# zzpDapeng/Transformer-Transducer

Hardware: AMD Instinct MI355X
Metric: utterances/sec (fwd+bwd) on 80-d fbank T=500 U=50 (higher is better)
Workload: dtype bf16

## Files before the change

### transformer-transducer_amd/csrc/gemm_fast.hip

```cpp
#include "gemm_fast.h"
#include "ttmi.h"
#include <mutex>

void ttmi_probe_begin(int slot, hipStream_t st);
void ttmi_probe_end(int slot, hipStream_t st);

namespace {

typedef float f32x16 __attribute__((ext_vector_type(16)));
typedef __bf16 bf16x8 __attribute__((ext_vector_type(8)));
typedef __bf16 bf16x4 __attribute__((ext_vector_type(4)));
typedef short s16x4 __attribute__((ext_vector_type(4)));

constexpr int TM = 128, TN_ = 128, TK = 64, NTH = 256;
constexpr int TILE_B = 128 * 64 * 2;
constexpr int GROUP_M = 8;

__device__ __attribute__((aligned(16))) const uint4 g_zero16 = {0u, 0u, 0u, 0u};

struct FP {
    const bf16_t* A;
    const bf16_t* B;
    void* C;
    const float* bias;
// ... 1622 lines not shown
        if (grp == 1) V9_BAR();
        int stg = 0;
        for (int t = 0; t < cnk; ++t) {
            const unsigned base = lds0 + stg * STG9;
#pragma unroll
            for (int ks = 0; ks < 2; ++ks) {
#pragma unroll
                for (int i = 0; i < 4; ++i) {
                    const unsigned a = base + aoff[i];
                    bf16x4 lo, hi;
                    if (ks == 0) { LDS_TR(lo, a, 0); LDS_TR(hi, a, 4 * 512); }
                    else { LDS_TR(lo, a, 32 * 512); LDS_TR(hi, a, 36 * 512); }
                    af[i][ks] = __builtin_shufflevector(lo, hi, 0, 1, 2, 3, 4, 5, 6, 7);
                }
#pragma unroll
                for (int i = 0; i < 4; ++i) {
                    const unsigned bq = base + boff[i];
                    bf16x4 lo, hi;
                    if (ks == 0) { LDS_TR(lo, bq, 0); LDS_TR(hi, bq, 4 * 256); }
                    else { LDS_TR(lo, bq, 32 * 256); LDS_TR(hi, bq, 36 * 256); }
                    bfr[i][ks] = __builtin_shufflevector(lo, hi, 0, 1, 2, 3, 4, 5, 6, 7);
                }
            }
            if (t + 2 < cnk) {
                TTMI_VM_GUARD("v9");
                stage(stg == 0 ? 2 : stg - 1, t + 2);
                TTMI_VM_WAIT("v9", V9_INFLIGHT);
            } else {
                asm volatile("s_waitcnt vmcnt(0)" ::: "memory");
            }
            asm volatile("s_waitcnt lgkmcnt(0)" ::: "memory");
            V9_BAR();
            __builtin_amdgcn_s_setprio(1);
#pragma unroll
            for (int ks = 0; ks < 2; ++ks)
#pragma unroll
                for (int mt = 0; mt < 4; ++mt)
#pragma unroll
                    for (int nt = 0; nt < 4; ++nt)
                        acc[mt][nt] = __builtin_amdgcn_mfma_f32_16x16x32_bf16(bfr[nt][ks], af[mt][ks], acc[mt][nt], 0, 0, 0);
            if (CS) {
#pragma unroll
                for (int mt = 0; mt < 4; ++mt)
#pragma unroll
                    for (int ks = 0; ks < 2; ++ks)
                        if (cs_unit == mt * 2 + ks) cs = __builtin_amdgcn_mfma_f32_16x16x32_bf16(ones, af[mt][ks], cs, 0, 0, 0);
            }
            __builtin_amdgcn_s_setprio(0);
            V9_BAR();
            stg = stg == 2 ? 0 : stg + 1;
        }
        if (grp == 0) V9_BAR();

        const int cbm = bm, cbn = bn, cunit = cs_unit;
        it += ncu;
        live = it < nitems;
        if (live) { item(it, bm, bn, tn); sources(bm, bn, kbeg); stage(0, 0); if (nk > 1) { TTMI_VM_GUARD("v9"); stage(1, 1); } }

        if (cnk > 0) {
            float* C = reinterpret_cast<float*>(p.C);
            float* img = reinterpret_cast<float*>(smem + 2 * STG9 + wave * 4096);
#pragma unroll
            for (int mi = 0; mi < 4; ++mi) {
#pragma unroll
                for (int ni = 0; ni < 4; ++ni)
                    *reinterpret_cast<f32x4*>(img + (lane & 15) * 64 + ((ni * 4 + (lane >> 4)) ^ (lane & 15)) * 4) = acc[mi][ni];
                const int n = cbn + wc * 64 + lane;
#pragma unroll
                for (int r = 0; r < 16; ++r) {
                    const int m = cbm + wr * 64 + mi * 16 + r;
                    const float v = img[r * 64 + (((lane >> 2) ^ r) << 2) + (lane & 3)];
                    if (m < p.M && n < p.N) atomicAdd(C + (long)m * p.ldc + n, v);
                }
            }
            if (CS && cunit >= 0 && lane < 16) {
                const int m = cbm + wr * 64 + (cunit >> 1) * 16 + lane;
                if (m < p.M) atomicAdd(p.colsum + m, cs[0]);
            }
        }
    }
#undef V9_BAR
}

struct TnGroupProb {
    const bf16_t* A; const bf16_t* B; float* C; float* colsum;
    int M, N, K, tiles_m;
    long lda, ldb, ldc;
    int tile0;
};
struct TnGroup {
    TnGroupProb pr[16];
    int n, total;
    int pieces;
};

__global__ __launch_bounds__(NTH8, 1) void gemm_tn_bf16_group_kernel(const TnGroup g) {
    extern __shared__ __attribute__((aligned(16))) char smem[];
    const unsigned lds0 = (unsigned)(size_t)smem;
    const int tid = threadIdx.x, lane = tid & 63, wave = __builtin_amdgcn_readfirstlane(tid >> 6);
    const int wr = wave & 3, wc = wave >> 2;
    const int grp = wave >> 2;
    const int xcd = blockIdx.x & 7, cu = blockIdx.x >> 3, ncu = gridDim.x >> 3;
    const int per_x = (g.total + 7) / 8;
    const int lo_x = min(xcd * per_x, g.total), hi = min((xcd + 1) * per_x, g.total);
    const int n_x = hi - lo_x, n_rounds = n_x / ncu, n_sur = n_x - n_rounds * ncu;
    const int P = (g.pieces && n_sur > 0 && 2 * n_sur <= ncu) ? ncu / n_sur : 0;
    const int n_whole = P ? n_rounds * ncu : n_x;
    const int n_items = n_whole + (P ? n_sur * P : 0);

    unsigned oA[4], oB[2];
    const char* baseA = nullptr;
    const char* baseB = nullptr;
    long lda = 0, ldb = 0;
    int nk = 0, q = 0;
    bool piece = false;
    auto item = [&](int v, int& bm, int& bn, int& tn) {
        piece = v >= n_whole;
        const int it = lo_x + (piece ? n_whole + (v - n_whole) / P : v);
        q = 0;
        while (q + 1 < g.n && it >= g.pr[q + 1].tile0) ++q;
        const TnGroupProb& pr = g.pr[q];
        const int t = it - pr.tile0;
        bm = (t % pr.tiles_m) * T9M;
        tn = t / pr.tiles_m;
        bn = tn * T9N;
        lda = pr.lda; ldb = pr.ldb;
        nk = pr.K / TK;
        baseA = reinterpret_cast<const char*>(pr.A);
        baseB = reinterpret_cast<const char*>(pr.B);
        if (piece) {
            const int part = (v - n_whole) % P;
            const long k0 = (long)part * nk / P, k1 = (long)(part + 1) * nk / P;
            baseA += k0 * TK * lda * 2;
            baseB += k0 * TK * ldb * 2;
            nk = (int)(k1 - k0);
        }
#pragma unroll
        for (int j = 0; j < 4; ++j) {
            const int k = (wave * 4 + j) * 2 + (lane >> 5);
            const int c = (lane & 31) ^ (((k & 3) << 2) | (((k >> 3) & 1) << 1));
            oA[j] = (unsigned)((k * lda + bm + c * 8) * 2);
        }
#pragma unroll
        for (int j = 0; j < 2; ++j) {
            const int k = (wave * 2 + j) * 4 + (lane >> 4);
            const int c = (lane & 15) ^ (((k & 3) << 2) | (((k >> 3) & 1) << 1));
            oB[j] = (unsigned)((k * ldb + bn + c * 8) * 2);
        }
    };
    auto stage = [&](int stg, int kt) {
        char* dst = smem + stg * STG9;
        const char* ba = baseA + (long)kt * TK * lda * 2;
        const char* bb = baseB + (long)kt * TK * ldb * 2;
#pragma unroll
        for (int j = 0; j < 4; ++j) glds16(ba + oA[j], dst + (wave * 4 + j) * 1024);
#pragma unroll
        for (int j = 0; j < 2; ++j) glds16(bb + oB[j], dst + T9M * 128 + (wave * 2 + j) * 1024);
    };

    const int gq = lane >> 4, qq = (lane >> 2) & 3, pp = lane & 3;
    const int swz = (qq << 2) | ((gq & 1) << 1);
    int aoff[4], boff[4];
#pragma unroll
    for (int i = 0; i < 4; ++i) {
        const int ca = wr * 64 + i * 16 + 4 * pp, cb = wc * 64 + i * 16 + 4 * pp;
        aoff[i] = (gq * 8 + qq) * 512 + (((ca >> 3) ^ swz) << 4) + (ca & 7) * 2;
        boff[i] = T9M * 128 + (gq * 8 + qq) * 256 + (((cb >> 3) ^ swz) << 4) + (cb & 7) * 2;
    }
    f32x4 acc[4][4];
    f32x4 cs = {0.f, 0.f, 0.f, 0.f};
    bf16x8 af[4][2], bfr[4][2];
    bf16x8 ones;
#pragma unroll
    for (int i = 0; i < 8; ++i) ones[i] = (__bf16)1.0f;
#define V9_BAR() __builtin_amdgcn_s_barrier()

    int bm = 0, bn = 0, tn = 0;
    int it = cu;
    bool live = it < n_items;
    if (live) { item(it, bm, bn, tn); stage(0, 0); if (nk > 1) { TTMI_VM_GUARD("v9"); stage(1, 1); } }
    while (live) {
#pragma unroll
        for (int i = 0; i < 4; ++i)
#pragma unroll
            for (int j = 0; j < 4; ++j) acc[i][j] = f32x4{0.f, 0.f, 0.f, 0.f};
        cs = f32x4{0.f, 0.f, 0.f, 0.f};
        const TnGroupProb cur = g.pr[q];
        const bool cpiece = piece;
        const int cs_mt = (cur.colsum && tn < 2) ? __builtin_amdgcn_readfirstlane(tn * 2 + wc) : -1;
        const int cnk = nk;
        if (cnk > 1) TTMI_VM_WAIT("v9", V9_INFLIGHT);
        else asm volatile("s_waitcnt vmcnt(0)" ::: "memory");
        V9_BAR();
        if (grp == 1) V9_BAR();
        int stg = 0;
        for (int t = 0; t < cnk; ++t) {
            const unsigned base = lds0 + stg * STG9;
#pragma unroll
            for (int ks = 0; ks < 2; ++ks) {
#pragma unroll
                for (int i = 0; i < 4; ++i) {
                    const unsigned a = base + aoff[i];
                    bf16x4 lo, hi2;
                    if (ks == 0) { LDS_TR(lo, a, 0); LDS_TR(hi2, a, 4 * 512); }
                    else { LDS_TR(lo, a, 32 * 512); LDS_TR(hi2, a, 36 * 512); }
                    af[i][ks] = __builtin_shufflevector(lo, hi2, 0, 1, 2, 3, 4, 5, 6, 7);
                }
#pragma unroll
                for (int i = 0; i < 4; ++i) {
                    const unsigned bq = base + boff[i];
                    bf16x4 lo, hi2;
                    if (ks == 0) { LDS_TR(lo, bq, 0); LDS_TR(hi2, bq, 4 * 256); }
                    else { LDS_TR(lo, bq, 32 * 256); LDS_TR(hi2, bq, 36 * 256); }
                    bfr[i][ks] = __builtin_shufflevector(lo, hi2, 0, 1, 2, 3, 4, 5, 6, 7);
                }
            }
            if (t + 2 < cnk) {
                TTMI_VM_GUARD("v9");
                stage(stg == 0 ? 2 : stg - 1, t + 2);
                TTMI_VM_WAIT("v9", V9_INFLIGHT);
            } else {
                asm volatile("s_waitcnt vmcnt(0)" ::: "memory");
            }
            asm volatile("s_waitcnt lgkmcnt(0)" ::: "memory");
            V9_BAR();
            __builtin_amdgcn_s_setprio(1);
#pragma unroll
            for (int ks = 0; ks < 2; ++ks)
#pragma unroll
                for (int mt = 0; mt < 4; ++mt)
#pragma unroll
                    for (int nt = 0; nt < 4; ++nt)
                        acc[mt][nt] = __builtin_amdgcn_mfma_f32_16x16x32_bf16(bfr[nt][ks], af[mt][ks], acc[mt][nt], 0, 0, 0);
#pragma unroll
            for (int mt = 0; mt < 4; ++mt)
                if (cs_mt == mt) {
                    cs = __builtin_amdgcn_mfma_f32_16x16x32_bf16(ones, af[mt][0], cs, 0, 0, 0);
                    cs = __builtin_amdgcn_mfma_f32_16x16x32_bf16(ones, af[mt][1], cs, 0, 0, 0);
                }
            __builtin_amdgcn_s_setprio(0);
// ... 356 lines not shown
    }
    int S = 1;
    bool strip_in = false;
    const bool tn8 = nbatch == 1 && accumulate && tn_v8_eligible(M, N, K, colsum_a != nullptr, &S, &strip_in);
    TTMI_REQUIRE(!colsum_w || tn8, "gemm_tn_bf16: weighted column sums exist on the persistent 256x256 kernel only (M=%d N=%d K=%d)", M, N, K);
    if (tn8) {
        const int ncu_x = g_num_cus / 8;
        p.tiles_m = M / T8; p.tiles_n = N / T8;
        const int nkt = cdiv(K, TK);
        const int Mfull = strip_in ? M : M / T8 * T8;
        p.M = Mfull; p.N = N; p.K = K; p.lda = lda; p.ldb = ldb; p.ldc = ldc;
        p.splitk = S; p.ksteps = cdiv(nkt, 8 * S); p.atomic = 1; p.gm = strip_in ? ncu_x / p.tiles_n : 0;
        if (colsum_a && p.csw) {
            if (int rc = enable_lds(gemm_tn_bf16_v8_kernel<2>, LDS8T)) return rc;
            hipLaunchKernelGGL(gemm_tn_bf16_v8_kernel<2>, dim3((unsigned)g_num_cus), dim3(NTH8), LDS8T, st, p);
        } else if (colsum_a) {
            if (int rc = enable_lds(gemm_tn_bf16_v8_kernel<1>, LDS8T)) return rc;
            hipLaunchKernelGGL(gemm_tn_bf16_v8_kernel<1>, dim3((unsigned)g_num_cus), dim3(NTH8), LDS8T, st, p);
        } else {
            if (int rc = enable_lds(gemm_tn_bf16_v8_kernel<0>, LDS8T)) return rc;
            hipLaunchKernelGGL(gemm_tn_bf16_v8_kernel<0>, dim3((unsigned)g_num_cus), dim3(NTH8), LDS8T, st, p);
        }
        TTMI_LAUNCH_CHECK("gemm_tn_bf16_v8_kernel");
        if (Mfull == M) return TTMI_OK;
        A += Mfull; C += (long)Mfull * ldc; M -= Mfull;
        if (colsum_a) colsum_a += Mfull;
        p.A = A; p.C = C; p.colsum = colsum_a;
    }
    p.M = M; p.N = N; p.K = K; p.lda = lda; p.ldb = ldb; p.ldc = ldc;
    p.tiles_m = cdiv(M, TM); p.tiles_n = cdiv(N, TN_);
    const long tiles = (long)p.tiles_m * p.tiles_n;
    const int ksteps_total = cdiv(K, TK);
    int splitk = 1;
    if (tiles * nbatch < 1024) {
        const long target = tiles * nbatch <= 16 && ksteps_total < 1024 ? std::min(g_tn_target_blocks, 256) : g_tn_target_blocks;
        splitk = (int)((target + tiles * nbatch - 1) / (tiles * nbatch));
        if (ksteps_total >= 1024 && splitk < 8) splitk = 8;
        if (splitk > ksteps_total / 4) splitk = ksteps_total / 4;
        if (splitk < 1) splitk = 1;
    }
    if (splitk >= 8) splitk = splitk / 8 * 8;
    p.ksteps = cdiv(ksteps_total, splitk);
    if (splitk < 8) splitk = cdiv(ksteps_total, p.ksteps);
    p.splitk = splitk;
    p.atomic = (splitk > 1 || accumulate) ? 1 : 0;
    p.gm = GROUP_M;
#define TN_LAUNCH(NB, CSF) hipLaunchKernelGGL((gemm_tn_bf16_kernel<NB, CSF>), dim3((unsigned)(tiles * splitk), nbatch), dim3(NTH), 2 * NB * TILE_B, st, p)
        if (g_gemm_fast_version >= 4) {
            if (colsum_a) TN_LAUNCH(1, true);
            else TN_LAUNCH(1, false);
        } else {
            if (colsum_a) TN_LAUNCH(2, true);
            else TN_LAUNCH(2, false);
        }
#undef TN_LAUNCH
    TTMI_LAUNCH_CHECK("gemm_tn_bf16_kernel");
    return TTMI_OK;
}

void gemm_fast_set_version(int v) {
    if (v == 14 || v == 15) { g_nt_stores = v == 15; return; }
    if (v >= 16) { g_bf16_mid = v - 16; return; }
    g_gemm_fast_version = v;
}
void gemm_fast_set_tn_target(int n) { g_tn_target_blocks = n; }
void gemm_fast_set_f32(int on) { g_f32_fast = on; }
int gemm_fast_f32_mode() { return g_f32_fast; }
void gemm_fast_set_reserved_cus(int n) { g_reserved_cus = n < 0 ? 0 : n; }
void gemm_fast_set_tn_group_pieces(int on) { g_tn_group_pieces = on; }
void gemm_fast_stream_reserve_cus(hipStream_t st, int n) {
    int dev = 0;
    (void)hipGetDevice(&dev);
    std::lock_guard<std::mutex> lock(g_res_mu);
    if (StreamRes* e = res_entry(dev, st, true)) { e->n = n < 0 ? 0 : n; e->has_n = true; }
}
void gemm_fast_alias_stream(hipStream_t child, hipStream_t parent) {
    int dev = 0;
    (void)hipGetDevice(&dev);
    std::lock_guard<std::mutex> lock(g_res_mu);
    if (StreamRes* e = res_entry(dev, child, true)) e->parent = parent;
}

bool gemm_tn_group_fits(const TnProblem& q) {
    return q.A && q.B && q.C && q.M > 0 && q.N > 0 && q.M % T9M == 0 && q.N % T9N == 0 && q.K % TK == 0 && q.K >= 2 * TK && q.lda % 8 == 0 && q.ldb % 8 == 0 && q.lda >= q.M && q.ldb >= q.N && q.ldc >= q.N &&
           aligned16(q.A) && aligned16(q.B) && (!q.colsum || q.N / T9N >= 2) && (long)q.K * q.lda * 2 < (1L << 32) && (long)q.K * q.ldb * 2 < (1L << 32);
}
int gemm_tn_bf16_group(const TnProblem* probs, int n, hipStream_t st) {
    TTMI_REQUIRE(probs && n >= 0, "gemm_tn_bf16_group: bad arguments");
    if (g_num_cus == 0) {
        int dev = 0, cnt = 0;
        if (hipGetDevice(&dev) == hipSuccess && hipDeviceGetAttribute(&cnt, hipDeviceAttributeMultiprocessorCount, dev) == hipSuccess && cnt > 0)
            g_num_cus = cnt / 8 * 8;
        if (g_num_cus <= 0) g_num_cus = 256;
    }
    if (int rc = enable_lds(gemm_tn_bf16_group_kernel, LDS9)) return rc;
    TnGroup g;
    g.n = 0; g.total = 0; g.pieces = 0;
    int min_nkt = 1 << 30;
    const int reserved = reserved_cus(st);
    const int cus = std::max(8, (g_num_cus - reserved) / 8 * 8);
    auto flush = [&]() -> int {
        if (g.n == 0) return TTMI_OK;
        g.pieces = reserved > 0 && min_nkt >= 2 * (cus / 8) && g_tn_group_pieces;
        min_nkt = 1 << 30;
        const bool probe = g.total >= 128;
        if (probe) ttmi_probe_begin(4, st);
        hipLaunchKernelGGL(gemm_tn_bf16_group_kernel, dim3((unsigned)cus), dim3(NTH8), LDS9, st, g);
        if (probe) ttmi_probe_end(4, st);
        TTMI_LAUNCH_CHECK("gemm_tn_bf16_group_kernel");
        g.n = 0; g.total = 0;
        return TTMI_OK;
    };
    for (int i = 0; i < n; ++i) {
        const TnProblem& q = probs[i];
        if (!gemm_tn_group_fits(q)) {
            if (int rc = gemm_tn_bf16(q.A, q.B, q.C, q.M, q.N, q.K, q.lda, q.ldb, q.ldc, 1, st, q.colsum)) return rc;
            continue;
        }
        TnGroupProb& d = g.pr[g.n];
        d.A = q.A; d.B = q.B; d.C = q.C; d.colsum = q.colsum; d.M = q.M; d.N = q.N; d.K = q.K; d.tiles_m = q.M / T9M;
        d.lda = q.lda; d.ldb = q.ldb; d.ldc = q.ldc; d.tile0 = g.total;
        g.total += d.tiles_m * (q.N / T9N);
        min_nkt = std::min(min_nkt, q.K / TK);
        if (++g.n == 16) { if (int rc = flush()) return rc; }
    }
    return flush();
}

extern "C" {
int ttmi_wgrad_group(const ttmi_wgrad_desc* descs, int n, void* stream) {
    static_assert(sizeof(ttmi_wgrad_desc) == sizeof(TnProblem), "ttmi_wgrad_desc and TnProblem must share one layout");
    return gemm_tn_bf16_group(reinterpret_cast<const TnProblem*>(descs), n, static_cast<hipStream_t>(stream));
}
int ttmi_gemm_nt_bf16(const void* A, const void* B, void* C, int c_dtype, const float* bias, int M, int N, int K, long lda,
                      long ldb, long ldc, void* stream) {
    NtEpilogue e;
    e.bias = bias;
    return gemm_nt_bf16(static_cast<const bf16_t*>(A), static_cast<const bf16_t*>(B), C, c_dtype, e, M, N, K, lda, ldb, ldc,
                        static_cast<hipStream_t>(stream), FastBatch());
}
int ttmi_gemm_nt_bf16_two_term(const void* A, const void* B, const void* B_lo, void* C, int c_dtype, const float* bias, int relu, int M, int N, int K,
                               long lda, long ldb, long ldc, void* stream) {
    NtEpilogue e;
    e.bias = bias; e.relu = relu; e.B_lo = static_cast<const bf16_t*>(B_lo);
    return gemm_nt_bf16(static_cast<const bf16_t*>(A), static_cast<const bf16_t*>(B), C, c_dtype, e, M, N, K, lda, ldb, ldc,
                        static_cast<hipStream_t>(stream), FastBatch());
}
int ttmi_gemm_nt_bf16_two_term_klo(const void* A, const void* B, const void* B_lo, void* C, int c_dtype, const float* bias, int relu, int M, int N, int K,
                                   int k_lo, long lda, long ldb, long ldc, void* stream) {
    NtEpilogue e;
    e.bias = bias; e.relu = relu; e.B_lo = static_cast<const bf16_t*>(B_lo); e.K_lo = k_lo;
    return gemm_nt_bf16(static_cast<const bf16_t*>(A), static_cast<const bf16_t*>(B), C, c_dtype, e, M, N, K, lda, ldb, ldc,
                        static_cast<hipStream_t>(stream), FastBatch());
}
int ttmi_gemm_nt_bf16_exp(const void* A, const void* B, void* C, const float* bias, float* rowsum, int nparts, const float* shift, int M, int N, int K,
                          long lda, long ldb, long ldc, void* stream) {
    NtEpilogue e;
    e.bias = bias; e.rowsum = rowsum; e.nparts = nparts; e.exp_shift = shift;
    return gemm_nt_bf16(static_cast<const bf16_t*>(A), static_cast<const bf16_t*>(B), C, 1, e, M, N, K, lda, ldb, ldc,
                        static_cast<hipStream_t>(stream), FastBatch());
}
int ttmi_gemm_nt_bf16_rowscale(const void* A, const void* B, void* C, void* mask, const float* rowscale, int M, int N, int K, long lda, long ldb, long ldc,
                               void* stream) {
    NtEpilogue e;
    e.mask = static_cast<const bf16_t*>(mask); e.mask_mode = 1; e.rowscale = rowscale;
    return gemm_nt_bf16(static_cast<const bf16_t*>(A), static_cast<const bf16_t*>(B), C, 1, e, M, N, K, lda, ldb, ldc,
                        static_cast<hipStream_t>(stream), FastBatch());
}
int ttmi_gemm_tn_bf16(const void* A, const void* B, float* C, int M, int N, int K, long lda, long ldb, long ldc, int accumulate,
                      float* colsum_a, void* stream) {
    return gemm_tn_bf16(static_cast<const bf16_t*>(A), static_cast<const bf16_t*>(B), C, M, N, K, lda, ldb, ldc, accumulate,
                        static_cast<hipStream_t>(stream), colsum_a, FastBatch());
}
int ttmi_gemm_tn_bf16_wsum(const void* A, const void* B, float* C, int M, int N, int K, long lda, long ldb, long ldc, float* colsum_a,
                           const void* colsum_w, void* stream) {
    return gemm_tn_bf16(static_cast<const bf16_t*>(A), static_cast<const bf16_t*>(B), C, M, N, K, lda, ldb, ldc, 1,
                        static_cast<hipStream_t>(stream), colsum_a, FastBatch(), static_cast<const bf16_t*>(colsum_w));
}
}
```

### transformer-transducer_amd/csrc/layers.hip

```cpp
#include "gemm.h"
#include "ttmi.h"
#include "rowops.h"
#include "gemm_fast.h"
#include "attn_flash.h"
#include <mutex>
#include <unordered_map>

void ttmi_probe_begin(int slot, hipStream_t st);
void ttmi_probe_end(int slot, hipStream_t st);
void ttmi_rnnt_set_lattice_version(int v);
void ttmi_rnnt_set_align_debug(int v);

namespace {

constexpr int NT_ = GEMM_A_KMAJOR | GEMM_B_KMAJOR;
constexpr int NN_ = GEMM_A_KMAJOR;
constexpr int TN_ = 0;

inline size_t al4(size_t n) { return (n + 3) & ~size_t(3); }

GemmDesc mk(const float* A, const float* B, float* C, int M, int N, int K, long lda, long ldb, long ldc, int flags, int prec) {
    GemmDesc d;
    d.A = A; d.B = B; d.C = C; d.M = M; d.N = N; d.K = K; d.lda = lda; d.ldb = ldb; d.ldc = ldc;
    d.flags = flags | (prec == 1 ? GEMM_BF16_MFMA : (prec == 2 ? GEMM_BF16X3 : 0));
// ... 854 lines not shown
    TTMI_REQUIRE(dz && y && w1 && w2 && ln_g && ctx && ws && (dy || skip_pre_norm) && g_w1 && g_b1 && g_w2 && g_b2 && g_ln_g && g_ln_b,
                 "ffn_bwd: null pointer");
    hipStream_t st = static_cast<hipStream_t>(stream);
    const bool fast = ffn_fast(prec, d, Di);
    TTMI_REQUIRE(!out || (fast && keep && aligned16(keep)), "ffn_bwd_defer: bf16 pipeline and a 16-byte aligned keep buffer required");
    Bump bc(const_cast<float*>(ctx)), bw(ws);
    FfnCtx c(bc, rows, d, Di, fast);
    FfnWs w(bw, rows, d, Di, fast, keep);
    DropSpec d_out, d_layer;
    d_out.p = p_drop; d_out.seed = seed ^ 0xC3u; d_out.salt = g_drop_salt;
    d_layer.p = p_layer; d_layer.seed = seed ^ 0xD4u; d_layer.salt = g_drop_salt;
    const float inv_keep = 1.f / (1.f - p_drop);
    CK(ln_bwd(dz, c.s2, c.mean2, c.rstd2, ln_g, nullptr, rows, d, w.dres, g_ln_g, g_ln_b, st, d_layer, fast ? w.dres16 : nullptr, d_out,
              fast ? g_b2 : nullptr));
    const float* df = w.dres;
    if (!fast) {
        if (p_drop > 0.f) {
            CK(dropout_apply(w.dres, rows * d, d_out, w.f, nullptr, st));
            df = w.f;
        }
        CK(colsum(df, d, rows, d, 1, 1, 0, 0, 0, 0, g_b2, st));
    }
    if (fast) {
        bf16_t* a1 = static_cast<bf16_t*>(c.a1);
        bf16_t* h = static_cast<bf16_t*>(c.h);
        bf16_t* da1 = static_cast<bf16_t*>(w.da1);
        int rc = TTMI_OK;
        const bf16_t* w1T16 = ctx_weightT(ctx, 0, w1, Di, d, Di, c.w1T16, st, &rc);
        CK(rc);
        const bf16_t* w2T16 = ctx_weightT(ctx, 1, w2, d, Di, d, c.w2T16, st, &rc);
        CK(rc);
        ctx_forget(ctx);
        if (out) out[0] = ttmi_wgrad_desc{w.dres16, a1, g_w2, nullptr, d, Di, (int)rows, (long)d, (long)Di, (long)Di};
        else CK(gemm_tn_bf16(w.dres16, a1, g_w2, d, Di, (int)rows, d, Di, Di, 1, fork_stream(st)));
        NtEpilogue e;
        e.mask = a1; e.scale = inv_keep;
        CK(gemm_nt_bf16(w.dres16, w2T16, da1, 1, e, (int)rows, Di, d, d, d, Di, st));
        if (out) out[1] = ttmi_wgrad_desc{da1, h, g_w1, g_b1, Di, d, (int)rows, (long)Di, (long)d, (long)d};
        else CK(gemm_tn_bf16(da1, h, g_w1, Di, d, (int)rows, Di, d, d, 1, fork_stream(st), g_b1));
        CK(gemm_nt_bf16(da1, w1T16, w.dh, 0, nullptr, (int)rows, d, Di, Di, Di, d, st));
    } else {
        const float* a1 = static_cast<const float*>(c.a1);
        const float* h = static_cast<const float*>(c.h);
        float* da1 = static_cast<float*>(w.da1);
        bf16_t* x3 = prec == 2 ? reinterpret_cast<bf16_t*>(ws + ((bw.floats() + 63) & ~(size_t)63)) : nullptr;
        if (x3 && x3_worth(rows, Di, d)) {
            CK(x3_tn(df, a1, g_w2, d, Di, rows, d, Di, Di, x3, st));
            CK(x3_nn(df, w2, da1, (int)rows, Di, d, d, Di, Di, NtEpilogue(), x3, st, true));
            CK(relu_mask_scale(da1, a1, rows * Di, inv_keep, st));
            CK(colsum(da1, Di, rows, Di, 1, 1, 0, 0, 0, 0, g_b1, st));
            CK(x3_tn(da1, h, g_w1, Di, d, rows, Di, d, d, x3, st));
            CK(x3_nn(da1, w1, w.dh, (int)rows, d, Di, Di, d, d, NtEpilogue(), x3, st, true));
        } else {
        CK(wgrad(df, a1, g_w2, d, Di, (int)rows, d, Di, Di, prec, st));
        GemmDesc g = mk(df, w2, da1, (int)rows, Di, d, d, Di, Di, NN_ | GEMM_MASK_AUX, prec);
        g.aux = a1; g.alpha = inv_keep;
        CK(ttmi_launch_gemm(g, st));
        CK(colsum(da1, Di, rows, Di, 1, 1, 0, 0, 0, 0, g_b1, st));
        CK(wgrad(da1, h, g_w1, Di, d, (int)rows, Di, d, d, prec, st));
        CK(ttmi_launch_gemm(mk(da1, w1, w.dh, (int)rows, d, Di, Di, d, d, NN_, prec), st));
        }
    }
    if (!skip_pre_norm) CK(ln_bwd(w.dh, y, c.mean1, c.rstd1, ln_g, w.dres, rows, d, dy, g_ln_g, g_ln_b, st));
    join_stream(st);
    return TTMI_OK;
}

int ttmi_ffn_bwd(const float* dz, const float* y, const float* w1, const float* w2, const float* ln_g, long rows, int d, int Di,
                 int prec, float p_drop, float p_layer, unsigned seed, const float* ctx, float* ws, float* dy, float* g_w1,
                 float* g_b1, float* g_w2, float* g_b2, float* g_ln_g, float* g_ln_b, void* stream) {
    return ffn_bwd_impl(dz, y, w1, w2, ln_g, rows, d, Di, prec, p_drop, p_layer, seed, ctx, ws, dy, g_w1, g_b1, g_w2, g_b2, g_ln_g, g_ln_b,
                        nullptr, nullptr, stream);
}
size_t ttmi_ffn_bwd_keep_bytes(long rows, int d, int Di) { return 2 * (keep_al((size_t)rows * Di) + keep_al((size_t)rows * d)); }
int ttmi_ffn_bwd_defer(const float* dz, const float* y, const float* w1, const float* w2, const float* ln_g, long rows, int d, int Di,
                       int prec, float p_drop, float p_layer, unsigned seed, const float* ctx, float* ws, float* dy, float* g_w1,
                       float* g_b1, float* g_w2, float* g_b2, float* g_ln_g, float* g_ln_b, void* keep, ttmi_wgrad_desc* out,
                       void* stream) {
    TTMI_REQUIRE(keep && out, "ffn_bwd_defer: keep buffer and descriptor array required");
    return ffn_bwd_impl(dz, y, w1, w2, ln_g, rows, d, Di, prec, p_drop, p_layer, seed, ctx, ws, dy, g_w1, g_b1, g_w2, g_b2, g_ln_g, g_ln_b,
                        keep, out, stream);
}
int ttmi_wgrad_defer_supported(long rows, int d, int H, int Dh, int Di, int prec) {
    return rows > 0 && attn_fast(prec, d, H, Dh) && ffn_fast(prec, d, Di) ? 1 : 0;
}

static size_t ws_round(size_t floats) { return (floats + 63) & ~size_t(63); }
int ttmi_layer_fused(int d, int H, int Dh, int Di, int prec) {
    return attn_fast(prec, d, H, Dh) && ffn_fast(prec, d, Di) && ln_bwd_pair_supported(d) ? 1 : 0;
}
size_t ttmi_layer_ws_floats(int B, int L, int d, int H, int Dh, int Di, int prec) {
    return ws_round(ttmi_attn_ws_floats(B, L, d, H, Dh, prec)) + ws_round(ttmi_ffn_ws_floats((long)B * L, d, Di, prec)) + ws_round((size_t)B * L * d) + 64;
}

int ttmi_layer_fwd(const float* x, const void* x16_in, const float* qkv_w, const float* o_w, const float* ln_g, const float* ln_b, const float* r_emb,
                   const float* r_w_bias, const float* r_bias, const float* w1, const float* b1, const float* w2, const float* b2,
                   const float* ff_ln_g, const float* ff_ln_b, int B, int L, int d, int H, int Dh, int K, int Di, int mask_kind, int mask_left,
                   int mask_right, const unsigned char* mask, long mask_sb, long mask_si, int prec, float p_drop_attn, unsigned seed_attn,
                   float p_drop_ffn, float p_layer, unsigned seed_ffn, float* ctx_attn, float* ctx_ffn, float* ws, float* y, float* z,
                   void* z16_out, void* stream) {
    TTMI_REQUIRE(ctx_attn && ctx_ffn && ws && y && z && ff_ln_g && ff_ln_b, "layer_fwd: null pointer");
    TTMI_REQUIRE(B > 0 && L > 0 && d > 0 && H > 0 && Dh > 0 && Di > 0, "layer_fwd: bad dims");
    TTMI_REQUIRE((reinterpret_cast<uintptr_t>(ctx_ffn) & 255) == 0, "layer_fwd: ctx_ffn must be 256-byte aligned");
    const bool fuse = ttmi_layer_fused(d, H, Dh, Di, prec) != 0;
    TTMI_REQUIRE(fuse || (!x16_in && !z16_out), "layer_fwd: bf16 copies of the residual stream exist in the fused bf16 pipeline only (ttmi_layer_fused)");
    const long rows = (long)B * L;
    float* ws_ffn = ws + ws_round(ttmi_attn_ws_floats(B, L, d, H, Dh, prec));
    LnPreNorm pre;
    if (fuse) {
        Bump bc(ctx_ffn);
        FfnCtx fc(bc, rows, d, Di, true);
        pre.g = ff_ln_g; pre.b = ff_ln_b; pre.h16 = static_cast<bf16_t*>(fc.h); pre.mean = fc.mean1; pre.rstd = fc.rstd1;
    }
    CK(attn_fwd_impl(x, qkv_w, o_w, ln_g, ln_b, r_emb, r_w_bias, r_bias, B, L, d, H, Dh, K, mask_kind, mask_left, mask_right, mask, mask_sb, mask_si,
                     prec, p_drop_attn, seed_attn, ctx_attn, ws, y, static_cast<const bf16_t*>(x16_in), fuse ? &pre : nullptr, stream));
    return ffn_fwd_impl(y, w1, b1, w2, b2, ff_ln_g, ff_ln_b, rows, d, Di, prec, p_drop_ffn, p_layer, seed_ffn, ctx_ffn, ws_ffn, z, fuse,
                        static_cast<bf16_t*>(z16_out), stream);
}

int ttmi_layer_bwd(const float* dz, const float* x, const void* x16_in, const float* y, const float* qkv_w, const float* o_w, const float* ln_g,
                   const float* r_emb, const float* r_w_bias, const float* r_bias, const float* w1, const float* w2, const float* ff_ln_g, int B,
                   int L, int d, int H, int Dh, int K, int Di, int mask_kind, int mask_left, int mask_right, const unsigned char* mask,
                   long mask_sb, long mask_si, int prec, float p_drop_attn, unsigned seed_attn, float p_drop_ffn, float p_layer,
                   unsigned seed_ffn, const float* ctx_attn, const float* ctx_ffn, float* ws, float* dx, float* g_qkv_w, float* g_o_w,
                   float* g_ln_g, float* g_ln_b, float* g_r_emb, float* g_r_w_bias, float* g_r_bias, float* g_w1, float* g_b1, float* g_w2,
                   float* g_b2, float* g_ff_ln_g, float* g_ff_ln_b, void* keep_attn, void* keep_ffn, ttmi_wgrad_desc* out, void* stream) {
    TTMI_REQUIRE(dz && x && y && ctx_attn && ctx_ffn && ws && dx, "layer_bwd: null pointer");
    TTMI_REQUIRE(B > 0 && L > 0 && d > 0 && H > 0 && Dh > 0 && Di > 0, "layer_bwd: bad dims");
    TTMI_REQUIRE((!out && !keep_attn && !keep_ffn) || (out && keep_attn && keep_ffn), "layer_bwd: keep buffers and descriptors come together");
    const bool fuse = ttmi_layer_fused(d, H, Dh, Di, prec) != 0;
    TTMI_REQUIRE(fuse || !x16_in, "layer_bwd: a bf16 copy of x exists in the fused bf16 pipeline only");
    const long rows = (long)B * L;
    float* ws_ffn = ws + ws_round(ttmi_attn_ws_floats(B, L, d, H, Dh, prec));
    float* dy = ws_ffn + ws_round(ttmi_ffn_ws_floats(rows, d, Di, prec));
    CK(ffn_bwd_impl(dz, y, w1, w2, ff_ln_g, rows, d, Di, prec, p_drop_ffn, p_layer, seed_ffn, ctx_ffn, ws_ffn, fuse ? nullptr : dy, g_w1, g_b1, g_w2,
                    g_b2, g_ff_ln_g, g_ff_ln_b, keep_ffn, out, stream, fuse));
    LnPairIn pair;
    if (fuse) {
        Bump bc(const_cast<float*>(ctx_ffn)), bw(ws_ffn);
        FfnCtx fc(bc, rows, d, Di, true);
        FfnWs fw(bw, rows, d, Di, true, keep_ffn);
        pair = LnPairIn{fw.dh, y, fc.mean1, fc.rstd1, ff_ln_g, fw.dres, g_ff_ln_g, g_ff_ln_b};
    }
    return attn_bwd_impl(fuse ? nullptr : dy, x, qkv_w, o_w, ln_g, r_emb, r_w_bias, r_bias, B, L, d, H, Dh, K, mask_kind, mask_left, mask_right, mask,
                         mask_sb, mask_si, prec, p_drop_attn, seed_attn, ctx_attn, ws, dx, g_qkv_w, g_o_w, g_ln_g, g_ln_b, g_r_emb, g_r_w_bias,
                         g_r_bias, keep_attn, out ? out + 2 : nullptr, stream, static_cast<const bf16_t*>(x16_in), fuse ? &pair : nullptr);
}

static inline bool joint_fast(int prec, int J) { return prec == 1 && J % 8 == 0; }
static inline size_t al8(size_t n) { return (n + 7) & ~(size_t)7; }
static inline bool joint_input_fast(int prec, int B, int T, int U1, int de, int dd, int J) {
    if (!joint_fast(prec, J) || de % 8 || dd % 8 || (long)B * T < 1024) return false;
    const size_t M = (size_t)B * T * U1, din = (size_t)de + dd;
    const size_t need = al8((size_t)B * T * de) + al8((size_t)B * U1 * dd) + al8((size_t)B * T * J) + 2 * al8((size_t)B * U1 * J) + al8(din * J) + 8;
    return need <= (size_t)M * J && need + al8(din * J) + al8((size_t)B * U1 * dd) <= 2 * (size_t)M * J;
}
int ttmi_joint_logits_dtype(int prec, int J) { return joint_fast(prec, J) ? 1 : 0; }

size_t ttmi_joint_ctx_floats(int B, int T, int U1, int J) { return al4(((size_t)B * T * U1 + 63) / 64 * 64 * J); }
size_t ttmi_joint_ctx_floats_prec(int B, int T, int U1, int J, int prec) {
    const size_t f = ttmi_joint_ctx_floats(B, T, U1, J);
    if (prec != 2) return f;
    const size_t x = al4((size_t)B * T * U1 * x3_pad(J) + 64);
    return x > f ? x : f;
}
static bool joint_x3_h3(long M, int V, int J) { return x3_worth(M, V, J) && J % 4 == 0; }
size_t ttmi_joint_ws_floats(int B, int T, int U1, int J, int V) {
// ... 423 lines not shown
```

### transformer-transducer_amd/tt/transformer.py

```python
import os

import torch
import torch.nn as nn

from ttmi import ops
from ttmi.ops import MaskSpec


def default_precision():
    v = os.environ.get("TTMI_PRECISION", "fp32").lower()
    return 1 if v in ("bf16", "1") else (2 if v in ("bf16x3", "2") else 0)


def label_precision():
    if default_precision() != 1:
        return None
    v = os.environ.get("TTMI_LABEL_PRECISION", "").lower()
    return 2 if v in ("bf16x3", "2") else (0 if v in ("fp32", "0") else None)


def label_value_precision():
    if default_precision() != 1:
        return None
    v = os.environ.get("TTMI_LABEL_VALUE_PRECISION", "bf16x3").lower()
    return 2 if v in ("bf16x3", "2") else (0 if v in ("fp32",) else None)


_mask_cache = {}


def as_mask_spec(mask, B, L):
    if mask is None:
        return MaskSpec(0)
    if isinstance(mask, MaskSpec):
        return mask
    ent = _mask_cache.get(id(mask))
    if ent is not None and ent[0]() is mask and ent[1] == mask._version:
        return ent[2]
    m = mask != 0
    if m.dim() == 2:
        t = m.t().unsqueeze(1)
    elif m.dim() == 3:
        t = m.permute(2, 0, 1)
    else:
        raise ValueError("attn_mask must be 2-D (klen, bsz) or 3-D (qlen, klen, bsz)")
    spec = MaskSpec(3, tensor=t.to(torch.uint8).contiguous())
    if t.is_cuda and t.shape[1] > 1:
        keep = ~t
        n = keep.sum(-1)
        lo = keep.int().argmax(-1)
        hi = t.shape[-1] - 1 - keep.flip(-1).int().argmax(-1)
        if bool(((n > 0) & (n == hi - lo + 1)).all()):
            rows = torch.arange(t.shape[1], device=t.device)
            reach = torch.stack([(rows - lo).max(), (hi - rows).max()]).clamp_(min=0).tolist()
            spec = MaskSpec(4, left=int(reach[0]), right=int(reach[1]), tensor=torch.stack([lo, hi], -1).to(torch.int32).contiguous())
    if len(_mask_cache) > 32:
        _mask_cache.clear()
    import weakref
    _mask_cache[id(mask)] = (weakref.ref(mask), mask._version, spec)
    return spec


def grad_targets(params, names, late=()):
    bufs, rets, after, later = {}, [], [], []
    for n, prm in zip(names, params):
        if getattr(prm, "_ttmi_direct", False) and prm.grad is not None:
            bufs[n] = prm.grad
            rets.append(None)
            cb = getattr(prm, "_ttmi_on_grad", None)
            if cb is not None:
                (later if n in late else after).append(cb)
        else:
            bufs[n] = torch.zeros_like(prm)
            rets.append(bufs[n])
    return (bufs, tuple(rets), after) if not late else (bufs, tuple(rets), after, later)


def _defer_queue(params, names, late, rows, prec, first_layer=False):
    q = ops.wgrad_queue
    if q is None or rows < 4096 or prec != 1 or (first_layer and q.immediate_first_layer):
        return None
    for n, prm in zip(names, params):
        if n in late and not (getattr(prm, "_ttmi_direct", False) and prm.grad is not None):
            return None
    return q


class _AttnFn(torch.autograd.Function):
    NAMES = ("qkv_w", "o_w", "ln_g", "ln_b", "r_emb", "r_w_bias", "r_bias")

    LATE = ("qkv_w", "o_w")

    @staticmethod
    def forward(ctx, x, qkv_w, o_w, ln_g, ln_b, r_emb, r_w_bias, r_bias, mask, prec, p_drop, seed, first_layer=False):
        x = x.contiguous()
        p = dict(zip(_AttnFn.NAMES, (t.detach() for t in (qkv_w, o_w, ln_g, ln_b, r_emb, r_w_bias, r_bias))))
        y, saved = ops.attn_fwd(x, p, mask, prec, p_drop, seed)
        ctx.save_for_backward(x, saved, *p.values())
        ctx.prec, ctx.p_drop, ctx.seed, ctx.mask, ctx.first_layer = prec, p_drop, seed, mask, first_layer
        ctx.params = (qkv_w, o_w, ln_g, ln_b, r_emb, r_w_bias, r_bias)
        return y

    @staticmethod
    def backward(ctx, dy):
        x, saved, *ps = ctx.saved_tensors
        p = dict(zip(_AttnFn.NAMES, ps))
        q = _defer_queue(ctx.params, _AttnFn.NAMES, _AttnFn.LATE, x.shape[0] * x.shape[1], ctx.prec, ctx.first_layer)
        if q is not None and ops.wgrad_defer_supported(x.shape[0] * x.shape[1], x.shape[2], p["r_emb"].shape[1], p["r_emb"].shape[2],
                                                      x.shape[2], ctx.prec):
            grads, rets, after, later = grad_targets(ctx.params, _AttnFn.NAMES, _AttnFn.LATE)
            dx = ops.attn_bwd(dy.contiguous(), x, p, saved, ctx.prec, grads, ctx.p_drop, ctx.seed, ctx.mask, defer=q)
            q.add_callbacks(later)
            q.maybe_flush(force=ctx.first_layer)
        else:
            grads, rets, after = grad_targets(ctx.params, _AttnFn.NAMES)
            dx = ops.attn_bwd(dy.contiguous(), x, p, saved, ctx.prec, grads, ctx.p_drop, ctx.seed, ctx.mask)
            if ctx.first_layer:
                ops.wgrad_flush()
        for cb in after:
            cb()
        return (dx, *rets, None, None, None, None, None)


class _FFNFn(torch.autograd.Function):
    NAMES = ("ff_w1", "ff_b1", "ff_w2", "ff_b2", "ff_ln_g", "ff_ln_b")

    @staticmethod
    def forward(ctx, y, w1, b1, w2, b2, ln_g, ln_b, prec, p_drop, p_layer, seed, first_layer=False):
        y = y.contiguous()
        p = dict(zip(_FFNFn.NAMES, (t.detach() for t in (w1, b1, w2, b2, ln_g, ln_b))))
        z, saved = ops.ffn_fwd(y, p, prec, p_drop, p_layer, seed)
        ctx.save_for_backward(y, saved, *p.values())
        ctx.prec, ctx.drop, ctx.first_layer = prec, (p_drop, p_layer, seed), first_layer
        ctx.params = (w1, b1, w2, b2, ln_g, ln_b)
        return z

    LATE = ("ff_w1", "ff_b1", "ff_w2")

    @staticmethod
    def backward(ctx, dz):
        y, saved, *ps = ctx.saved_tensors
        p = dict(zip(_FFNFn.NAMES, ps))
        rows = y.numel() // y.shape[-1]
        if ctx.first_layer and ops.wgrad_queue is not None and ops.wgrad_queue.immediate_first_layer:
            ops.wgrad_flush()
        q = _defer_queue(ctx.params, _FFNFn.NAMES, _FFNFn.LATE, rows, ctx.prec, ctx.first_layer)
        if q is not None and ops.wgrad_defer_supported(rows, y.shape[-1], 1, 8, p["ff_w1"].shape[0], ctx.prec):
            grads, rets, after, later = grad_targets(ctx.params, _FFNFn.NAMES, _FFNFn.LATE)
            dy = ops.ffn_bwd(dz.contiguous(), y, p, saved, ctx.prec, grads, *ctx.drop, defer=q)
            q.add_callbacks(later)
        else:
            grads, rets, after = grad_targets(ctx.params, _FFNFn.NAMES)
            dy = ops.ffn_bwd(dz.contiguous(), y, p, saved, ctx.prec, grads, *ctx.drop)
        for cb in after:
            cb()
        return (dy, *rets, None, None, None, None, None)


_SUBLAYER_CALLS = bool(os.environ.get("TTMI_SUBLAYER_CALLS"))


class _LayerFn(torch.autograd.Function):
    NAMES = _AttnFn.NAMES + _FFNFn.NAMES
# ... 137 lines not shown
```

### transformer-transducer_amd/ttmi/ops.py

```python
import ctypes
import math
import os
import sys

import torch

from . import check, lib

c_int, c_long, c_float, c_void_p = ctypes.c_int, ctypes.c_long, ctypes.c_float, ctypes.c_void_p


_TRACE = bool(os.environ.get("TTMI_TRACE_CALLS"))


def _trace(name, *dims):
    if _TRACE:
        print("[ttmi] %s %s stream %x" % (name, dims, torch.cuda.current_stream().cuda_stream), file=sys.stderr, flush=True)


def _p(t):
    return c_void_p(t.data_ptr()) if t is not None else c_void_p(0)


def _stream():
# ... 102 lines not shown
    return ld


def ctc_loss_fwd(logits, labels, act_lens, label_lens, blank, workspace):
    _need_cuda(logits, labels, act_lens, label_lens, workspace)
    ld = _ctc_args(logits, labels)
    B, T, V = logits.shape
    costs = torch.empty(B, dtype=torch.float32, device=logits.device)
    check(lib().ttmi_ctc_loss_fwd(_p(logits), c_long(ld), _p(labels), _p(act_lens), _p(label_lens), c_int(B), c_int(T), c_int(labels.shape[1]),
                                  c_int(V), c_int(blank), _p(workspace), _p(costs), _stream()), "ttmi_ctc_loss_fwd")
    return costs


def ctc_loss_bwd(logits, labels, act_lens, label_lens, blank, workspace, grad_out, grad_out_stride, scale, inplace=False):
    _need_cuda(logits, labels, act_lens, label_lens, workspace, grad_out)
    ld = _ctc_args(logits, labels)
    B, T, V = logits.shape
    if inplace:
        grad = logits
    elif ld == V:
        grad = torch.empty_like(logits)
    else:
        grad = torch.empty(B, T, ld, dtype=logits.dtype, device=logits.device)[..., :V]
    check(lib().ttmi_ctc_loss_bwd(_p(logits), c_long(ld), _p(labels), _p(act_lens), _p(label_lens), c_int(B), c_int(T), c_int(labels.shape[1]),
                                  c_int(V), c_int(blank), _p(workspace), _p(grad_out), c_int(grad_out_stride), c_float(scale), _p(grad),
                                  c_long(ld), _stream()), "ttmi_ctc_loss_bwd")
    return grad


def ctc_greedy(logits, act_lens, blank=0):
    _need_cuda(logits, act_lens)
    if logits.dim() != 3 or logits.dtype is not torch.float32 or row_pitch(logits) is None:
        raise ValueError("ctc_greedy: logits must be f32 [B, T, V], dense or row-padded")
    B, T, V = logits.shape
    tokens = torch.empty(B, T, dtype=torch.int32, device=logits.device)
    count = torch.empty(B, dtype=torch.int32, device=logits.device)
    check(lib().ttmi_ctc_greedy(_p(logits), c_long(row_pitch(logits)), _p(act_lens), c_int(B), c_int(T), c_int(V), c_int(blank), _p(tokens),
                                _p(count), _stream()), "ttmi_ctc_greedy")
    return tokens, count


def linear_nt(x, w, out, bias=None, prec=0, accumulate=False):
    M, K = x.shape
    N = w.shape[0]
    flags = GEMM_A_KMAJOR | GEMM_B_KMAJOR | (GEMM_BIAS if bias is not None else 0) | _PREC_FLAG[prec]
    return gemm(x, w, out, M, N, K, x.stride(0), w.stride(0), out.stride(0), flags, bias=bias, beta=1.0 if accumulate else 0.0)


def linear_nn(g, w, out, prec=0):
    M, N = g.shape
    K = w.shape[1]
    return gemm(g, w, out, M, K, N, g.stride(0), w.stride(0), out.stride(0), GEMM_A_KMAJOR | _PREC_FLAG[prec])


def linear_tn(g, x, out, prec=0, accumulate=True):
    M, N = g.shape
    K = x.shape[1]
    return gemm(g, x, out, N, K, M, g.stride(0), x.stride(0), out.stride(0) if out.dim() == 2 else 1, _PREC_FLAG[prec],
                beta=1.0 if accumulate else 0.0)


GEMM_BIAS, GEMM_RELU, GEMM_ATOMIC, GEMM_MASK_AUX, GEMM_A_KMAJOR, GEMM_B_KMAJOR, GEMM_BF16_MFMA, GEMM_BF16X3 = 1, 2, 4, 8, 16, 32, 64, 128
_DT = {torch.float32: 0, torch.bfloat16: 1}
_PREC_FLAG = {0: 0, 1: GEMM_BF16_MFMA, 2: GEMM_BF16X3}


def gemm(A, B, C, M, N, K, lda, ldb, ldc, flags, bias=None, aux=None, alpha=1.0, beta=0.0, nz1=1, nz2=1,
         sA=(0, 0), sB=(0, 0), sC=(0, 0), splitk=1):
    _need_cuda(A, B, C, bias, aux)
    check(lib().ttmi_gemm(_p(A), _p(B), _p(C), _p(bias), _p(aux), c_int(_DT[A.dtype]), c_int(_DT[B.dtype]),
                          c_int(_DT[C.dtype]), c_int(M), c_int(N), c_int(K), c_long(lda), c_long(ldb), c_long(ldc),
                          c_int(nz1), c_int(nz2), c_long(sA[0]), c_long(sA[1]), c_long(sB[0]), c_long(sB[1]),
                          c_long(sC[0]), c_long(sC[1]), c_float(alpha), c_float(beta), c_int(flags), c_int(splitk),
                          _stream()), "ttmi_gemm")
    return C


class WgradDesc(ctypes.Structure):
    _fields_ = [("A", c_void_p), ("B", c_void_p), ("C", c_void_p), ("colsum", c_void_p), ("M", c_int), ("N", c_int), ("K", c_int),
                ("lda", c_long), ("ldb", c_long), ("ldc", c_long)]


class _WgradLane:
    __slots__ = ("stream", "descs", "alive", "after")

    def __init__(self, stream):
        self.stream, self.descs, self.alive, self.after = stream, [], [], []


class WgradQueue:

    def __init__(self, group=4, immediate_first_layer=False):
        self.limit = 4 * group
        self.immediate_first_layer = immediate_first_layer
        self.lanes = {}

    def _lane(self):
        st = torch.cuda.current_stream()
        key = (st.device.index, st.cuda_stream)
        lane = self.lanes.get(key)
        if lane is None:
            lane = self.lanes[key] = _WgradLane(st)
        return lane

    @property
    def descs(self):
        return self._lane().descs

    def push(self, descs, tensors):
        lane = self._lane()
        lane.descs.extend(WgradDesc.from_buffer_copy(d) for d in descs)
        lane.alive.append(tensors)

    def add_callbacks(self, cbs):
        self._lane().after.extend(cbs)

    def maybe_flush(self, force=False):
        lane = self._lane()
        if lane.descs and (force or len(lane.descs) >= self.limit):
            arr = (WgradDesc * len(lane.descs))(*lane.descs)
            check(lib().ttmi_wgrad_group(arr, c_int(len(lane.descs)), _stream()), "ttmi_wgrad_group")
            cbs = lane.after
            lane.descs, lane.alive, lane.after = [], [], []
            for cb in cbs:
                cb()

    def flush_all(self):
        for lane in list(self.lanes.values()):
            if lane.descs:
                with torch.cuda.stream(lane.stream):
                    self.maybe_flush(force=True)

    def discard(self):
        self.lanes = {}


wgrad_queue = None


def wgrad_defer_supported(rows, d, H, Dh, Di, prec):
    return bool(lib().ttmi_wgrad_defer_supported(c_long(rows), c_int(d), c_int(H), c_int(Dh), c_int(Di), c_int(prec)))


def wgrad_flush(every_stream=False):
    if wgrad_queue is not None:
        if every_stream:
            wgrad_queue.flush_all()
        else:
            wgrad_queue.maybe_flush(force=True)


class MaskSpec:
    __slots__ = ("kind", "left", "right", "tensor")

    def __init__(self, kind=0, left=None, right=None, tensor=None):
        unknown = -1 if kind == 4 else 0
        self.kind, self.tensor = kind, tensor
        self.left = unknown if left is None else left
        self.right = unknown if right is None else right

    def args(self):
        t = self.tensor
        if self.kind == 4:
            return c_int(4), c_int(self.left), c_int(self.right), _p(t), c_long(t.stride(0) if t.shape[0] > 1 else 0), c_long(2)
        if self.kind != 3:
            return c_int(self.kind), c_int(self.left), c_int(self.right), c_void_p(0), c_long(0), c_long(0)
        sb = t.stride(0) if t.shape[0] > 1 else 0
        si = t.stride(1) if t.shape[1] > 1 else 0
        return c_int(3), c_int(0), c_int(0), _p(t), c_long(sb), c_long(si)


def _f32(n, device):
    return torch.empty(int(n), dtype=torch.float32, device=device)


_ws_cache = {}
_side_streams = {}


def scratch(n, device):
    key = (device.type, device.index, torch.cuda.current_stream(device).cuda_stream)
    t = _ws_cache.get(key)
    if t is None or t.numel() < n:
        t = _ws_cache[key] = _f32(max(int(n), 1 << 20), device)
    return t


def scratch_generation(device, stream):
    t = _ws_cache.get((device.type, device.index, stream.cuda_stream))
    return None if t is None else t.data_ptr()


def attn_fwd(x, p, mask, prec, p_drop=0.0, seed=0):
    _trace("attn_fwd", tuple(x.shape))
    _need_cuda(x)
    B, L, d = x.shape
    K, H, Dh = p["r_emb"].shape
    L_ = lib()
    L_.ttmi_attn_ctx_floats.restype = ctypes.c_size_t
    L_.ttmi_attn_ws_floats.restype = ctypes.c_size_t
    ctx = _f32(L_.ttmi_attn_ctx_floats(c_int(B), c_int(L), c_int(d), c_int(H), c_int(Dh), c_int(prec)), x.device)
    ws = scratch(L_.ttmi_attn_ws_floats(c_int(B), c_int(L), c_int(d), c_int(H), c_int(Dh), c_int(prec)), x.device)
    y = torch.empty_like(x)
    check(L_.ttmi_attn_fwd(_p(x), _p(p["qkv_w"]), _p(p["o_w"]), _p(p["ln_g"]), _p(p["ln_b"]), _p(p["r_emb"]),
                           _p(p["r_w_bias"]), _p(p["r_bias"]), c_int(B), c_int(L), c_int(d), c_int(H), c_int(Dh), c_int(K),
                           *mask.args(), c_int(prec), c_float(p_drop), ctypes.c_uint(seed), _p(ctx), _p(ws), _p(y), _stream()),
# ... 517 lines not shown
```

Before: 1039.

## Defer and batch short-row weight-gradient GEMMs into grouped TN launches

Weight-gradient GEMMs for layers with fewer than 4096 rows were previously computed immediately. They now go through the deferred wgrad queue, which holds them until a forced flush so many small problems share one grouped launch. To allow this, the grouped TN kernel accepts K that is only a multiple of 8. Partial K tiles are zero-filled by redirecting loads past the valid rows to a zero page, and the group capacity rises from 16 to 24. The trade-off is held memory for the queued activations, extra masking arithmetic in the staging loop, and coarse per-wave row masking granularity.

```diff
diff --git a/transformer-transducer_amd/csrc/gemm_fast.hip b/transformer-transducer_amd/csrc/gemm_fast.hip
--- a/transformer-transducer_amd/csrc/gemm_fast.hip
+++ b/transformer-transducer_amd/csrc/gemm_fast.hip
@@ -1728,6 +1728,8 @@
 #undef V9_BAR
 }
 
+constexpr int TN_GROUP_MAX = 24;
+__device__ __attribute__((aligned(128))) const unsigned g_tn_zero_page[32] = {};
 struct TnGroupProb {
     const bf16_t* A; const bf16_t* B; float* C; float* colsum;
     int M, N, K, tiles_m;
@@ -1735,7 +1737,7 @@
     int tile0;
 };
 struct TnGroup {
-    TnGroupProb pr[16];
+    TnGroupProb pr[TN_GROUP_MAX];
     int n, total;
     int pieces;
 };
@@ -1759,6 +1761,7 @@
     const char* baseB = nullptr;
     long lda = 0, ldb = 0;
     int nk = 0, q = 0;
+    int krows = 0;
     bool piece = false;
     auto item = [&](int v, int& bm, int& bn, int& tn) {
         piece = v >= n_whole;
@@ -1771,7 +1774,8 @@
         tn = t / pr.tiles_m;
         bn = tn * T9N;
         lda = pr.lda; ldb = pr.ldb;
-        nk = pr.K / TK;
+        nk = (pr.K + TK - 1) / TK;
+        krows = pr.K;
         baseA = reinterpret_cast<const char*>(pr.A);
         baseB = reinterpret_cast<const char*>(pr.B);
         if (piece) {
@@ -1780,6 +1784,7 @@
             baseA += k0 * TK * lda * 2;
             baseB += k0 * TK * ldb * 2;
             nk = (int)(k1 - k0);
+            krows = pr.K - (int)k0 * TK;
         }
 #pragma unroll
         for (int j = 0; j < 4; ++j) {
@@ -1798,10 +1803,15 @@
         char* dst = smem + stg * STG9;
         const char* ba = baseA + (long)kt * TK * lda * 2;
         const char* bb = baseB + (long)kt * TK * ldb * 2;
-#pragma unroll
-        for (int j = 0; j < 4; ++j) glds16(ba + oA[j], dst + (wave * 4 + j) * 1024);
-#pragma unroll
-        for (int j = 0; j < 2; ++j) glds16(bb + oB[j], dst + T9M * 128 + (wave * 2 + j) * 1024);
+        const unsigned long long keep = wave * 8 < krows - kt * TK ? ~0ull : 0ull;
+        const unsigned long long zp = reinterpret_cast<unsigned long long>(g_tn_zero_page);
+        const char* sa = reinterpret_cast<const char*>(zp + ((reinterpret_cast<unsigned long long>(ba) - zp) & keep));
+        const char* sb = reinterpret_cast<const char*>(zp + ((reinterpret_cast<unsigned long long>(bb) - zp) & keep));
+        const unsigned ko = (unsigned)keep;
+#pragma unroll
+        for (int j = 0; j < 4; ++j) glds16(sa + (oA[j] & ko), dst + (wave * 4 + j) * 1024);
+#pragma unroll
+        for (int j = 0; j < 2; ++j) glds16(sb + (oB[j] & ko), dst + T9M * 128 + (wave * 2 + j) * 1024);
     };
 
     const int gq = lane >> 4, qq = (lane >> 2) & 3, pp = lane & 3;
@@ -2324,7 +2334,7 @@
 }
 
 bool gemm_tn_group_fits(const TnProblem& q) {
-    return q.A && q.B && q.C && q.M > 0 && q.N > 0 && q.M % T9M == 0 && q.N % T9N == 0 && q.K % TK == 0 && q.K >= 2 * TK && q.lda % 8 == 0 && q.ldb % 8 == 0 && q.lda >= q.M && q.ldb >= q.N && q.ldc >= q.N &&
+    return q.A && q.B && q.C && q.M > 0 && q.N > 0 && q.M % T9M == 0 && q.N % T9N == 0 && q.K % 8 == 0 && q.K >= 8 && q.lda % 8 == 0 && q.ldb % 8 == 0 && q.lda >= q.M && q.ldb >= q.N && q.ldc >= q.N &&
            aligned16(q.A) && aligned16(q.B) && (!q.colsum || q.N / T9N >= 2) && (long)q.K * q.lda * 2 < (1L << 32) && (long)q.K * q.ldb * 2 < (1L << 32);
 }
 int gemm_tn_bf16_group(const TnProblem* probs, int n, hipStream_t st) {
@@ -2344,8 +2354,8 @@
     auto flush = [&]() -> int {
         if (g.n == 0) return TTMI_OK;
         g.pieces = reserved > 0 && min_nkt >= 2 * (cus / 8) && g_tn_group_pieces;
+        const bool probe = g.total >= 128 && min_nkt >= 64;
         min_nkt = 1 << 30;
-        const bool probe = g.total >= 128;
         if (probe) ttmi_probe_begin(4, st);
         hipLaunchKernelGGL(gemm_tn_bf16_group_kernel, dim3((unsigned)cus), dim3(NTH8), LDS9, st, g);
         if (probe) ttmi_probe_end(4, st);
@@ -2363,8 +2373,8 @@
         d.A = q.A; d.B = q.B; d.C = q.C; d.colsum = q.colsum; d.M = q.M; d.N = q.N; d.K = q.K; d.tiles_m = q.M / T9M;
         d.lda = q.lda; d.ldb = q.ldb; d.ldc = q.ldc; d.tile0 = g.total;
         g.total += d.tiles_m * (q.N / T9N);
-        min_nkt = std::min(min_nkt, q.K / TK);
-        if (++g.n == 16) { if (int rc = flush()) return rc; }
+        min_nkt = std::min(min_nkt, (q.K + TK - 1) / TK);
+        if (++g.n == TN_GROUP_MAX) { if (int rc = flush()) return rc; }
     }
     return flush();
 }
diff --git a/transformer-transducer_amd/csrc/layers.hip b/transformer-transducer_amd/csrc/layers.hip
--- a/transformer-transducer_amd/csrc/layers.hip
+++ b/transformer-transducer_amd/csrc/layers.hip
@@ -960,7 +960,7 @@
                         keep, out, stream);
 }
 int ttmi_wgrad_defer_supported(long rows, int d, int H, int Dh, int Di, int prec) {
-    return rows > 0 && attn_fast(prec, d, H, Dh) && ffn_fast(prec, d, Di) ? 1 : 0;
+    return rows > 0 && (rows >= 4096 || rows % 8 == 0) && attn_fast(prec, d, H, Dh) && ffn_fast(prec, d, Di) ? 1 : 0;
 }
 
 static size_t ws_round(size_t floats) { return (floats + 63) & ~size_t(63); }
diff --git a/transformer-transducer_amd/tt/transformer.py b/transformer-transducer_amd/tt/transformer.py
--- a/transformer-transducer_amd/tt/transformer.py
+++ b/transformer-transducer_amd/tt/transformer.py
@@ -78,7 +78,7 @@
 
 def _defer_queue(params, names, late, rows, prec, first_layer=False):
     q = ops.wgrad_queue
-    if q is None or rows < 4096 or prec != 1 or (first_layer and q.immediate_first_layer):
+    if q is None or prec != 1 or (first_layer and q.immediate_first_layer):
         return None
     for n, prm in zip(names, params):
         if n in late and not (getattr(prm, "_ttmi_direct", False) and prm.grad is not None):
diff --git a/transformer-transducer_amd/ttmi/ops.py b/transformer-transducer_amd/ttmi/ops.py
--- a/transformer-transducer_amd/ttmi/ops.py
+++ b/transformer-transducer_amd/ttmi/ops.py
@@ -208,13 +208,15 @@
 
 
 class _WgradLane:
-    __slots__ = ("stream", "descs", "alive", "after")
+    __slots__ = ("stream", "descs", "alive", "after", "hold")
 
     def __init__(self, stream):
-        self.stream, self.descs, self.alive, self.after = stream, [], [], []
+        self.stream, self.descs, self.alive, self.after, self.hold = stream, [], [], [], False
 
 
 class WgradQueue:
+
+    SHORT_ROWS = 4096
 
     def __init__(self, group=4, immediate_first_layer=False):
         self.limit = 4 * group
@@ -237,17 +239,18 @@
         lane = self._lane()
         lane.descs.extend(WgradDesc.from_buffer_copy(d) for d in descs)
         lane.alive.append(tensors)
+        lane.hold = lane.hold or any(d.K < self.SHORT_ROWS for d in descs)
 
     def add_callbacks(self, cbs):
         self._lane().after.extend(cbs)
 
     def maybe_flush(self, force=False):
         lane = self._lane()
-        if lane.descs and (force or len(lane.descs) >= self.limit):
+        if lane.descs and (force or (len(lane.descs) >= self.limit and not lane.hold)):
             arr = (WgradDesc * len(lane.descs))(*lane.descs)
             check(lib().ttmi_wgrad_group(arr, c_int(len(lane.descs)), _stream()), "ttmi_wgrad_group")
             cbs = lane.after
-            lane.descs, lane.alive, lane.after = [], [], []
+            lane.descs, lane.alive, lane.after, lane.hold = [], [], [], False
             for cb in cbs:
                 cb()
 
```

Result: no change. 1043 (median of 6 runs) (+0.4%).
